# YyzHarry/imbalanced-regression

Hardware: NVIDIA B200
Metric: images/sec (higher is better)
Workload: dtype bf16

## Files before the change

### imbalanced-regression_b200/csrc/conv.cuh

```cuda
#pragma once
#include "common.cuh"

namespace dirb200 {

struct ConvShape {
  int n, h, w, cin, cout, kh, kw, stride, pad, ho, wo;
};

struct StatLayout {
  int rows, n_tiles, bn, group;
};

int conv_fprop(const __nv_bfloat16* x, const __nv_bfloat16* w, __nv_bfloat16* y, const ConvShape& s, bool stem,
               cudaStream_t st, float* stat_partial = nullptr, StatLayout* layout = nullptr);
struct ConvEpilogue {
  const float* scale;
  const float* shift;
  const __nv_bfloat16* residual;
  bool relu;
};
int conv_fprop_affine(const __nv_bfloat16* x, const __nv_bfloat16* w, __nv_bfloat16* out, const ConvShape& s,
                      const ConvEpilogue& epi, cudaStream_t st);
struct DgradBnMoments {
  const __nv_bfloat16* y;
  const float *scale, *shift;
  float* partial;
  StatLayout* layout;
};
bool conv_dgrad_fuses_bn_moments(const ConvShape& s);
int conv_dgrad(const __nv_bfloat16* dy, const __nv_bfloat16* wt, __nv_bfloat16* dx, const ConvShape& s,
               cudaStream_t st, const DgradBnMoments* bnm = nullptr);
int conv_wgrad_splits(const ConvShape& s);
size_t conv_wgrad_workspace_bytes(const ConvShape& s);
int conv_wgrad_partials(const __nv_bfloat16* x, const __nv_bfloat16* dy, float* partial, const ConvShape& s, bool stem,
                        int* splits_out, cudaStream_t st);
int wgrad_reduce(const float* workspace, int splits, float* dw, const ConvShape& s, bool stem, bool accumulate,
                 cudaStream_t st);
int conv_wgrad(const __nv_bfloat16* x, const __nv_bfloat16* dy, float* dw, float* workspace, const ConvShape& s,
               bool stem, bool accumulate, cudaStream_t st);
struct WgradReduceDesc {
  const float* partial;
  size_t w_off;
  int splits, cout, cin, kh, kw, stem;
};
int wgrad_reduce_all(const WgradReduceDesc* descs_dev, int nlayers, float* grads, cudaStream_t st);
struct PrepDesc {
  size_t w_off;
  int cout, cin, kh, kw, stem;
  __nv_bfloat16 *wf, *wd;
  FastDiv fd_cin, fd_cout, fd_taps;
// ... 17 lines not shown
```

### imbalanced-regression_b200/csrc/conv_igemm.cu

```cuda
#include <stdlib.h>
#include "common.cuh"
#include "tc.cuh"
#include "conv.cuh"

namespace dirb200 {
using namespace tc;

constexpr int BM = 128;
constexpr int BK = 64;
constexpr int kProducerThreads = 128;
constexpr int kTmaWarp = 4, kMmaWarp = 5;
constexpr int kThreads = 320;
constexpr int kMaxTaps = 25;

struct IgemmParams {
  const __nv_bfloat16* src;
  int n, hs, ws, cs;
  int hm, wm;
  int kh, kw, stride, pad;
  int transposed;
  int cls_on, cls_py, cls_px, full_h, full_w;
  int ntaps_c;
  int tap_list[kMaxTaps];
  long long tap_eoff[kMaxTaps];
  unsigned short tap_r[kMaxTaps], tap_s[kMaxTaps];
  FastDiv fd_hw, fd_wm, fd_cpb, fd_kw, fd_ntiles, fd_persplit;
  int cpb;
  long long pixels;
  int num_kblocks;
  int kblocks_per_split;
  int total_chunks;
  int m_tiles, n_tiles;
  int num_tiles;
  int a_mode;
  int i2c_stride, i2c_lo;
  int ldc;
  void* out;
  float* stat_out;
  const float* epi_scale;
  const float* epi_shift;
  const __nv_bfloat16* epi_res;
  int epi_relu;
  const __nv_bfloat16* bst_y;
  const float* bst_scale;
  const float* bst_shift;
  int patch_r, patch_wp, patch_h, patch_w;
  FastDiv fd_tpi, fd_wp;
};

template <int BN, bool STAGED_EPI, bool CTA2 = false, bool PATCH = false>
struct Cfg {
  static constexpr int kABytes = BM * BK * 2;
  static constexpr int kBRows = CTA2 ? BN / 2 : BN;
  static constexpr int kBBytes = kBRows * BK * 2;
  static constexpr int kStageBytes = PATCH ? 32768 : kABytes + kBBytes;
  static constexpr int kBresBytes = PATCH ? 9 * BN * BK * 2 : 0;
  static constexpr int kEpiCols = 64;
  static constexpr int kStages = PATCH ? 3
                                 : CTA2 ? ((BN == 256) ? 6 : 8)
                                        : (STAGED_EPI ? ((BN == 256) ? 4 : ((BN == 128) ? 6 : 8))
                                                      : ((BN == 256) ? 4 : ((BN == 128) ? 6 : 8)));
// ... 41 lines not shown
}

__device__ __forceinline__ const __nv_bfloat16* tap_source(const IgemmParams& P, const RowPre& rp, int r, int s,
                                                           int coff, bool& ok) {
  int hi, wi;
  ok = true;
  if (!P.transposed) {
    hi = rp.yb + r;
    wi = rp.xb + s;
  } else {
    hi = rp.yb - r;
    wi = rp.xb - s;
    if (P.stride == 2) {
      ok = ((hi | wi) & 1) == 0;
      hi >>= 1;
      wi >>= 1;
    }
  }
  ok = ok && static_cast<unsigned>(hi) < static_cast<unsigned>(P.hs) &&
       static_cast<unsigned>(wi) < static_cast<unsigned>(P.ws);
  return ok ? P.src + (static_cast<size_t>(rp.nb + hi) * P.ws + wi) * P.cs + coff : P.src;
}

template <int BN, bool WGRAD, bool STEM, bool CTA2 = false, bool ATMA = false, bool AFFINE = false, bool BSTAT = false,
          bool PATCH = false>
__global__ void __launch_bounds__((ATMA && !PATCH) ? kThreads - kProducerThreads : kThreads, 1)
igemm_kernel(const __grid_constant__ CUtensorMap tmap_b, const __grid_constant__ CUtensorMap tmap_a,
             const IgemmParams P) {
  using C = Cfg<BN, !WGRAD, CTA2, PATCH>;
  static_assert(!PATCH || (ATMA && !WGRAD && !CTA2 && !AFFINE && BN == 64), "patch-resident A operand: 64-wide fprop / dgrad");
  static_assert(!CTA2 || (ATMA && !WGRAD && !STEM && BN >= 128), "CTA pairs: TMA-fed fprop / dgrad GEMMs only");
  static_assert(!ATMA || !STEM, "TMA-fed A operand: not for the stem");
  static_assert(!AFFINE || (ATMA && !WGRAD), "folded-BN epilogue: TMA-fed fprop GEMMs only");
  static_assert(!BSTAT || (ATMA && !WGRAD && !AFFINE), "BN-backward moments in the epilogue: TMA-fed dgrad GEMMs only");
  extern __shared__ uint8_t smem_raw[];
  const uint32_t smem_base = (smem_u32(smem_raw) + 1023u) & ~1023u;
  const uint32_t bar_base = smem_base + C::kBarOffset;
  auto a_addr = [&](int s) { return smem_base + s * C::kStageBytes; };
  auto b_addr = [&](int s) { return smem_base + s * C::kStageBytes + C::kABytes; };
  constexpr uint32_t nstages = C::kStages;
  auto full_bar = [&](int s) { return bar_base + 8u * s; };
  auto empty_bar = [&](int s) { return bar_base + 8u * (C::kStages + s); };
  auto tfull_bar = [&](int a) { return bar_base + 8u * (2 * C::kStages + a); };
  auto tempty_bar = [&](int a) { return bar_base + 8u * (2 * C::kStages + 2 + a); };
  const uint32_t tmem_holder = bar_base + 8u * (2 * C::kStages + 4);
  const uint32_t bres_bar = bar_base + 8u * (2 * C::kStages + 5);
  const uint32_t bres_addr = smem_base + C::kBresOffset;

  const int warp = static_cast<int>(threadIdx.x >> 5) + ((ATMA && !PATCH) ? kProducerThreads / 32 : 0), lane = threadIdx.x & 31;
  const uint32_t rank = CTA2 ? cluster_ctarank() : 0u;
  const int tile_start = CTA2 ? static_cast<int>(blockIdx.x >> 1) : static_cast<int>(blockIdx.x);
// ... 603 lines not shown
      if (lane == 0) {
        if (CTA2 && rank != 0) mbar_arrive_remote(mapa_rank(tempty_bar(acc), 0));
        else mbar_arrive(tempty_bar(acc));
      }
    }
    if constexpr (!WGRAD) {
      if (P.stat_out != nullptr) {
        __syncwarp();
        if constexpr (PATCH) asm volatile("bar.sync 1, 256;" ::: "memory");
        else asm volatile("bar.sync 1, 128;" ::: "memory");
        const float* all = reinterpret_cast<const float*>(smem_raw + (smem_base - smem_u32(smem_raw)) + C::kStatOffset);
        constexpr int kWarpFloats = C::kStatWarpBytes / 4;
        float* dst = P.stat_out + static_cast<size_t>(blockIdx.x) * 2 * P.ldc + fixed_n * BN;
        if (egroup == 0) {
          for (int o = quarter * 32 + lane; o < 2 * BN; o += 128) {
            const int k = o / BN, col = o - k * BN;
            const int cb = col / C::kEpiCols, ln = (col % C::kEpiCols) >> 1, e = col & 1;
            const int idx = (cb * 4 + k * 2 + e) * 32 + ln;
            float v = (all[idx] + all[kWarpFloats + idx]) + (all[2 * kWarpFloats + idx] + all[3 * kWarpFloats + idx]);
            if constexpr (PATCH)
              v += (all[4 * kWarpFloats + idx] + all[5 * kWarpFloats + idx]) + (all[6 * kWarpFloats + idx] + all[7 * kWarpFloats + idx]);
            dst[static_cast<size_t>(k) * P.ldc + col] = v;
          }
        }
      }
    }
  }

  tcgen05_fence_before();
  __syncwarp();
  if constexpr (CTA2) cluster_sync_all();
  else __syncthreads();
  if (warp == kMmaWarp) {
    tcgen05_fence_after();
    if constexpr (CTA2) tmem_dealloc_cta2(tmem_base, C::kTmemCols);
    else tmem_dealloc(tmem_base, C::kTmemCols);
  }
}


constexpr int kWgpThreads = 192;
constexpr int kWgpStages = 4, kWgpASlot = 32768, kWgpBSlot = 16384, kWgpStage = kWgpASlot + kWgpBSlot;
constexpr int kWgpSmemBytes = kWgpStages * kWgpStage + 256 + 1024;

__global__ void __launch_bounds__(kWgpThreads, 1)
wgrad_patch_kernel(const __grid_constant__ CUtensorMap tmap_x, const __grid_constant__ CUtensorMap tmap_dy,
                   const IgemmParams P) {
  extern __shared__ uint8_t smem_raw[];
  const uint32_t smem_base = (smem_u32(smem_raw) + 1023u) & ~1023u;
  const uint32_t bar_base = smem_base + kWgpStages * kWgpStage;
  auto a_addr = [&](int s) { return smem_base + s * kWgpStage; };
  auto b_addr = [&](int s) { return smem_base + s * kWgpStage + kWgpASlot; };
  auto full_bar = [&](int s) { return bar_base + 8u * s; };
  auto empty_bar = [&](int s) { return bar_base + 8u * (kWgpStages + s); };
  const uint32_t done_bar = bar_base + 8u * (2 * kWgpStages), tmem_holder = bar_base + 8u * (2 * kWgpStages + 1);
  const int warp = threadIdx.x >> 5, lane = threadIdx.x & 31;

  for (int i = threadIdx.x; i < kWgpStages * kWgpStage / 16; i += kWgpThreads)
    asm volatile("st.shared.v4.b32 [%0], {%1, %1, %1, %1};" ::"r"(smem_base + i * 16), "r"(0u) : "memory");
// ... 389 lines not shown
    set_error("cuTensorMapEncodeTiled (patch) failed (%d) w=%d h=%d n=%d rows=%d", (int)cr, w, h, n, box_rows);
    return DIRB200_ERR_CUDA;
  }
  return DIRB200_OK;
}

static int launch_patch(const __nv_bfloat16* src, const __nv_bfloat16* wmat, IgemmParams P, int n, int h, int w, int r,
                        bool flipped, cudaStream_t st) {
  CUtensorMap ta, tb;
  if (int rc = make_tmap_patch(&ta, src, n, h, w, r + 2)) return rc;
  if (int rc = make_tmap_bf16_2d(&tb, wmat, 9 * 64, 64, 9 * 64 * 2, 64)) return rc;
  P.patch_r = r; P.patch_wp = w + 2; P.patch_h = h; P.patch_w = w;
  P.transposed = flipped ? 1 : 0;
  P.a_mode = 3;
  P.n_tiles = 1;
  P.m_tiles = n * (h / r);
  P.num_tiles = P.m_tiles;
  P.num_kblocks = 9;
  if (P.bst_y != nullptr) return launch_igemm_impl<64, false, false, true, false, true, true>(tb, ta, P, st);
  return launch_igemm_impl<64, false, false, true, false, false, true>(tb, ta, P, st);
}

static int conv_fprop_impl(const __nv_bfloat16* x, const __nv_bfloat16* w, __nv_bfloat16* y, const ConvShape& s, bool stem,
                           cudaStream_t st, float* stat_partial, const ConvEpilogue* epi);

int conv_fprop(const __nv_bfloat16* x, const __nv_bfloat16* w, __nv_bfloat16* y, const ConvShape& s, bool stem,
               cudaStream_t st, float* stat_partial, StatLayout* layout) {
  const int rc = conv_fprop_impl(x, w, y, s, stem, st, stat_partial, nullptr);
  if (layout) *layout = t_last_layout;
  return rc;
}

int conv_fprop_affine(const __nv_bfloat16* x, const __nv_bfloat16* w, __nv_bfloat16* out, const ConvShape& s,
                      const ConvEpilogue& epi, cudaStream_t st) {
  DIRB_CHECK_ARG(epi.scale && epi.shift, "conv_fprop_affine: scale / shift missing");
  return conv_fprop_impl(x, w, out, s, false, st, nullptr, &epi);
}

static int conv_fprop_impl(const __nv_bfloat16* x, const __nv_bfloat16* w, __nv_bfloat16* y, const ConvShape& s, bool stem,
                           cudaStream_t st, float* stat_partial, const ConvEpilogue* epi) {
  if (int rc = check_shape(s, stem, "conv_fprop")) return rc;
  const int ktot = s.kh * s.kw * s.cin;
  IgemmParams P{};
  P.src = x; P.n = s.n; P.hs = s.h; P.ws = s.w; P.cs = s.cin; P.hm = s.ho; P.wm = s.wo;
  P.kh = s.kh; P.kw = s.kw; P.stride = s.stride; P.pad = s.pad; P.transposed = 0;
  P.cpb = stem ? 1 : s.cin / 64;
  P.pixels = static_cast<long long>(s.n) * s.ho * s.wo;
  P.num_kblocks = ktot / 64;
  P.ntaps_c = s.kh * s.kw;
  DIRB_CHECK_ARG(stem || P.ntaps_c <= kMaxTaps, "conv_fprop: at most %d filter taps (got %dx%d)", kMaxTaps, s.kh, s.kw);
  for (int i = 0; i < kMaxTaps; ++i) P.tap_list[i] = i;
  P.ldc = s.cout; P.out = y;
  P.stat_out = stat_partial;
  if (epi) {
    P.epi_scale = epi->scale; P.epi_shift = epi->shift; P.epi_res = epi->residual; P.epi_relu = epi->relu ? 1 : 0;
  }
  if (!stem && !epi) {
    if (const int pr = patch_rows(s.h, s.w, s.cin, s.kh, s.kw, s.stride, s.pad, s.cout))
      return launch_patch(x, w, P, s.n, s.h, s.w, pr, false, st);
  }
  const int m_tiles = static_cast<int>((P.pixels + BM - 1) / BM);
  const int bn = pick_bn(s.cout, m_tiles, !is_plain_gemm(s, stem));
  P.n_tiles = s.cout / bn;
  CUtensorMap tm, ta;
  bool tma_fed = false;
  if (is_plain_gemm(s, stem)) {
    if (int rc = make_tmap_bf16_2d(&ta, x, s.cin, static_cast<uint64_t>(P.pixels), static_cast<uint64_t>(s.cin) * 2, BM))
      return rc;
    P.a_mode = 1;
    tma_fed = true;
  } else if (!stem && im2col_enabled()) {
    if (int rc = make_tmap_im2col_bf16(&ta, x, s.cin, s.w, s.h, s.n, -s.pad, -s.pad, s.pad - (s.kw - 1),
                                       s.pad - (s.kh - 1), s.stride, BM))
      return rc;
    P.a_mode = 2; P.i2c_stride = s.stride; P.i2c_lo = -s.pad;
    tma_fed = true;
  }
  if (tma_fed && want_pairs(bn, P.num_kblocks)) return launch_cta2(w, ktot, s.cout, P, m_tiles, st, ta);
  if (int rc = make_tmap_bf16_2d(&tm, w, ktot, s.cout, static_cast<uint64_t>(ktot) * 2, bn)) return rc;
  if (stem) return DISPATCH_BN(bn, false, true, tm, P, m_tiles, 1, st);
  if (tma_fed) return DISPATCH_BN(bn, false, false, tm, P, m_tiles, 1, st, &ta);
  return DISPATCH_BN(bn, false, false, tm, P, m_tiles, 1, st);
}

bool conv_dgrad_fuses_bn_moments(const ConvShape& s) {
  return s.stride == 1 && (is_plain_gemm(s, false) || (im2col_enabled() && s.kh == s.kw));
}

int conv_dgrad(const __nv_bfloat16* dy, const __nv_bfloat16* wt, __nv_bfloat16* dx, const ConvShape& s,
               cudaStream_t st, const DgradBnMoments* bnm) {
  if (int rc = check_shape(s, false, "conv_dgrad")) return rc;
  DIRB_CHECK_ARG(!bnm || (conv_dgrad_fuses_bn_moments(s) && bnm->y && bnm->scale && bnm->shift && bnm->partial),
                 "conv_dgrad: BN-backward moments are fused into TMA-fed stride-1 dgrads only");
  DIRB_CHECK_ARG(s.stride == 1 || s.stride == 2, "conv_dgrad: stride must be 1 or 2 (got %d)", s.stride);
  DIRB_CHECK_ARG(s.kh * s.kw <= (s.stride == 1 ? kMaxTaps : 9), "conv_dgrad: at most %d filter taps (stride 2: 9; got %dx%d)",
                 kMaxTaps, s.kh, s.kw);
  const int ktot = s.kh * s.kw * s.cout;
  IgemmParams P{};
  P.src = dy; P.n = s.n; P.hs = s.ho; P.ws = s.wo; P.cs = s.cout; P.hm = s.h; P.wm = s.w;
  P.kh = s.kh; P.kw = s.kw; P.stride = s.stride; P.pad = s.pad; P.transposed = 1;
  P.cpb = s.cout / 64;
  P.ldc = s.cin; P.out = dx;
  if (bnm) {
    P.bst_y = bnm->y; P.bst_scale = bnm->scale; P.bst_shift = bnm->shift; P.stat_out = bnm->partial;
  }
  CUtensorMap tm;
  if (s.stride == 1) {
    P.pixels = static_cast<long long>(s.n) * s.h * s.w;
    P.ntaps_c = s.kh * s.kw;
    for (int i = 0; i < kMaxTaps; ++i) P.tap_list[i] = i;
    P.num_kblocks = ktot / 64;
    if (const int pr = patch_rows(s.ho, s.wo, s.cout, s.kh, s.kw, s.stride, s.pad, s.cin)) {
      const int rc = launch_patch(dy, wt, P, s.n, s.ho, s.wo, pr, true, st);
      if (bnm && bnm->layout) *bnm->layout = t_last_layout;
      return rc;
    }
    const int m_tiles = static_cast<int>((P.pixels + BM - 1) / BM);
    const int bn = pick_bn(s.cin, m_tiles, !is_plain_gemm(s, false));
    P.n_tiles = s.cin / bn;
    CUtensorMap ta;
    bool tma_fed = false;
    if (is_plain_gemm(s, false)) {
      if (int rc = make_tmap_bf16_2d(&ta, dy, s.cout, static_cast<uint64_t>(P.pixels), static_cast<uint64_t>(s.cout) * 2, BM))
        return rc;
      P.a_mode = 1;
      tma_fed = true;
    } else if (im2col_enabled() && s.kh == s.kw) {
// ... 217 lines not shown
```

### imbalanced-regression_b200/csrc/nn_kernels.cu

```cuda
#include "common.cuh"
#include "conv.cuh"
#include "nn.cuh"

namespace dirb200 {

constexpr int kReduceCtasPerSm = 4;

struct V8 {
  float v[8];
};
__device__ __forceinline__ V8 load8(const __nv_bfloat16* p) {
  const uint4 u = *reinterpret_cast<const uint4*>(p);
  const __nv_bfloat162* h = reinterpret_cast<const __nv_bfloat162*>(&u);
  V8 r;
#pragma unroll
  for (int i = 0; i < 4; ++i) {
    const float2 f = __bfloat1622float2(h[i]);
    r.v[2 * i] = f.x;
    r.v[2 * i + 1] = f.y;
  }
  return r;
}
__device__ __forceinline__ void store8(__nv_bfloat16* p, const V8& a) {
  uint4 u;
  __nv_bfloat162* h = reinterpret_cast<__nv_bfloat162*>(&u);
// ... 77 lines not shown
#pragma unroll
    for (int u = 0; u < 4; ++u) x[u] = load8(y + (r + u * stride) * c + cg * 8);
#pragma unroll
    for (int u = 0; u < 4; ++u)
#pragma unroll
      for (int j = 0; j < 8; ++j) {
        acc[0][j] += x[u].v[j];
        acc[1][j] = fmaf(x[u].v[j], x[u].v[j], acc[1][j]);
      }
  }
  for (; r < rows; r += stride) {
    const V8 x = load8(y + r * c + cg * 8);
#pragma unroll
    for (int j = 0; j < 8; ++j) {
      acc[0][j] += x.v[j];
      acc[1][j] = fmaf(x.v[j], x.v[j], acc[1][j]);
    }
  }
  column_reduce_finish<2>(acc, cg, cgroups, c, partial);
}

__device__ __forceinline__ void sum_layout2(const float* __restrict__ partial, const StatLayout& L, int c, int i,
                                            double (*sh)[32][32], double& r0, double& r1) {
  double a0 = 0.0, b0 = 0.0, a1 = 0.0, b1 = 0.0;
  if (i < c) {
    const int j = i / L.bn;
    const int ngroups = L.rows / L.group;
    const int nk = j < ngroups ? (ngroups - 1 - j) / L.n_tiles + 1 : 0;
    const int nrows = nk * L.group;
    int t = threadIdx.y;
    for (; t + 32 < nrows; t += 64) {
      const int q0 = (j + (t / L.group) * L.n_tiles) * L.group + t % L.group;
      const int q1 = (j + ((t + 32) / L.group) * L.n_tiles) * L.group + (t + 32) % L.group;
      const float x0 = partial[((size_t)q0 * 2) * c + i], y0 = partial[((size_t)q0 * 2 + 1) * c + i];
      const float x1 = partial[((size_t)q1 * 2) * c + i], y1 = partial[((size_t)q1 * 2 + 1) * c + i];
      a0 += (double)x0; b0 += (double)y0; a1 += (double)x1; b1 += (double)y1;
    }
    if (t < nrows) {
      const int q0 = (j + (t / L.group) * L.n_tiles) * L.group + t % L.group;
      a0 += (double)partial[((size_t)q0 * 2) * c + i];
      b0 += (double)partial[((size_t)q0 * 2 + 1) * c + i];
    }
  }
  sh[0][threadIdx.y][threadIdx.x] = a0 + a1;
  sh[1][threadIdx.y][threadIdx.x] = b0 + b1;
  __syncthreads();
  r0 = r1 = 0.0;
  if (threadIdx.y == 0)
    for (int w = 0; w < 32; ++w) {
      r0 += sh[0][w][threadIdx.x];
      r1 += sh[1][w][threadIdx.x];
    }
}

__global__ void bn_finalize_kernel(const float* __restrict__ partial, StatLayout L, int64_t rows, int c,
                                   const float* __restrict__ gamma, const float* __restrict__ beta, float eps,
                                   float momentum, float* __restrict__ running_mean, float* __restrict__ running_var,
                                   float* __restrict__ mean_out, float* __restrict__ invstd_out,
                                   float* __restrict__ scale, float* __restrict__ shift) {
  __shared__ double sh[2][32][32];
  const int i = blockIdx.x * 32 + threadIdx.x;
  double sx, sq;
  sum_layout2(partial, L, c, i, sh, sx, sq);
  if (threadIdx.y != 0 || i >= c) return;
  const double n = (double)rows;
  const double m = sx / n;
  double var = sq / n - m * m;
  if (var < 0.0) var = 0.0;
  const float invstd = (float)(1.0 / sqrt(var + (double)eps));
  mean_out[i] = (float)m;
  invstd_out[i] = invstd;
  const float sc = gamma[i] * invstd;
  scale[i] = sc;
  shift[i] = beta[i] - (float)m * sc;
  if (running_mean) {
    const double unbiased = rows > 1 ? var * n / (n - 1.0) : var;
    running_mean[i] = (1.f - momentum) * running_mean[i] + momentum * (float)m;
    running_var[i] = (1.f - momentum) * running_var[i] + momentum * (float)unbiased;
  }
}

__global__ void bn_eval_coeffs_kernel(int c, const float* __restrict__ gamma, const float* __restrict__ beta, float eps,
                                      const float* __restrict__ running_mean, const float* __restrict__ running_var,
                                      float* __restrict__ scale, float* __restrict__ shift) {
  const int i = blockIdx.x * blockDim.x + threadIdx.x;
  if (i >= c) return;
  const float sc = gamma[i] * rsqrtf(running_var[i] + eps);
  scale[i] = sc;
  shift[i] = beta[i] - running_mean[i] * sc;
}

__global__ void bn_eval_coeffs_all_kernel(const BnEvalDesc* __restrict__ descs, const float* __restrict__ params,
                                          const float* __restrict__ running, float eps) {
  const BnEvalDesc d = descs[blockIdx.y];
  const int i = blockIdx.x * blockDim.x + threadIdx.x;
  if (i >= d.c) return;
  const float sc = params[d.gamma_off + i] * rsqrtf(running[d.rv_off + i] + eps);
  d.scale[i] = sc;
  d.shift[i] = params[d.beta_off + i] - running[d.rm_off + i] * sc;
}

__device__ __forceinline__ uint32_t f2_to_bf2(float a, float b) {
// ... 166 lines not shown
        const float2 yv = bf2_to_f2(yw[w]);
        ms.apply(M[u], w, yv, g);
        if (WRITE_DZ) {
          oz[w] = f2_to_bf2(g.x, g.y);
          g = bf2_to_f2(oz[w]);
        }
        acc[0][2 * w] += g.x;
        acc[0][2 * w + 1] += g.y;
        acc[1][2 * w] = fmaf(g.x, yv.x, acc[1][2 * w]);
        acc[1][2 * w + 1] = fmaf(g.y, yv.y, acc[1][2 * w + 1]);
        if (HAS_Y2) {
          const uint32_t y2w[4] = {Y2[u].x, Y2[u].y, Y2[u].z, Y2[u].w};
          const float2 y2v = bf2_to_f2(y2w[w]);
          acc[K - 1][2 * w] = fmaf(g.x, y2v.x, acc[K - 1][2 * w]);
          acc[K - 1][2 * w + 1] = fmaf(g.y, y2v.y, acc[K - 1][2 * w + 1]);
        }
      }
      if (WRITE_DZ) *reinterpret_cast<uint4*>(dz_out + (u ? o1 : o0)) = make_uint4(oz[0], oz[1], oz[2], oz[3]);
    }
  }
  column_reduce_finish<K>(acc, cg, cgroups, c, partial);
}

__device__ __forceinline__ void bn_bwd_coeffs_write(double db, double s1, int i, int64_t rows, int c,
                                                    const float* __restrict__ mean, const float* __restrict__ invstd,
                                                    const float* __restrict__ gamma, float* __restrict__ grad_gamma,
                                                    float* __restrict__ grad_beta, float* __restrict__ coef) {
  const double n = (double)rows, is = (double)invstd[i], ga = (double)gamma[i], mu = (double)mean[i];
  const double dg = is * (s1 - mu * db);
  coef[i] = (float)(ga * is);
  coef[c + i] = (float)(-ga * is * is * dg / n);
  coef[2 * c + i] = (float)(ga * is * (mu * is * dg / n - db / n));
  grad_gamma[i] += (float)dg;
  grad_beta[i] += (float)db;
}

__global__ void bn_bwd_coeffs_kernel(const float* __restrict__ partial, int nblocks, int K, int gslot, int64_t rows,
                                     int c, const float* __restrict__ mean, const float* __restrict__ invstd,
                                     const float* __restrict__ gamma, float* __restrict__ grad_gamma,
                                     float* __restrict__ grad_beta, float* __restrict__ coef ) {
  __shared__ double sh[32][32];
  const int i = blockIdx.x * 32 + threadIdx.x;
  double db, s1;
  sum_partials2(partial, nblocks, K, 0, gslot, c, i, sh, db, s1);
  if (threadIdx.y != 0 || i >= c) return;
  bn_bwd_coeffs_write(db, s1, i, rows, c, mean, invstd, gamma, grad_gamma, grad_beta, coef);
}

__global__ void bn_bwd_coeffs_layout_kernel(const float* __restrict__ partial, StatLayout L, int64_t rows, int c,
                                            const float* __restrict__ mean, const float* __restrict__ invstd,
                                            const float* __restrict__ gamma, float* __restrict__ grad_gamma,
                                            float* __restrict__ grad_beta, float* __restrict__ coef) {
  __shared__ double sh[2][32][32];
  const int i = blockIdx.x * 32 + threadIdx.x;
  double db, s1;
  sum_layout2(partial, L, c, i, sh, db, s1);
  if (threadIdx.y != 0 || i >= c) return;
  bn_bwd_coeffs_write(db, s1, i, rows, c, mean, invstd, gamma, grad_gamma, grad_beta, coef);
}
// ... 781 lines not shown
```

### imbalanced-regression_b200/csrc/resnet_runner.cu

```cuda
#include <stdlib.h>
#include <vector>
#include "common.cuh"
#include "conv.cuh"
#include "nn.cuh"

namespace dirb200 {

struct BNLayer {
  int c = 0;
  size_t gamma_off = 0, beta_off = 0;
  size_t rm_off = 0, rv_off = 0;
  float *mean = nullptr, *invstd = nullptr, *scale = nullptr, *shift = nullptr, *coef = nullptr;
};

struct ConvLayer {
  ConvShape s{};
  bool stem = false;
  size_t w_off = 0;
  __nv_bfloat16 *wf = nullptr, *wd = nullptr;
  float* wpart = nullptr;
  __nv_bfloat16* y = nullptr;
  __nv_bfloat16* a = nullptr;
  int64_t rows = 0;
  BNLayer bn;
// ... 4 lines not shown
  bool has_ds = false;
  const __nv_bfloat16* in = nullptr;
  __nv_bfloat16* out = nullptr;
  uint8_t* mask = nullptr;
};

}

using namespace dirb200;

struct dirb200_net {
  int n = 0, h = 0, w = 0;
  ConvLayer stem;
  std::vector<Block> blocks;
  __nv_bfloat16 *x_s2d = nullptr, *pool_out = nullptr;
  uint8_t* pool_idx = nullptr;
  int pool_h = 0, pool_w = 0;
  int feat_c = 0, feat_hw = 0;
  __nv_bfloat16* scratch[8] = {};
  WgradReduceDesc* reduce_descs = nullptr;
  std::vector<int> reduce_begin;
  float* bn_partial = nullptr;
  float* stat_partial = nullptr;
  PrepDesc* prep_descs = nullptr;
  BnEvalDesc* bn_eval_descs = nullptr;
  int num_bns = 0, max_bn_c = 0;
  int num_convs = 0;
  size_t param_count = 0, running_count = 0, activation_bytes = 0;
  std::vector<void*> allocs;
  bool forward_was_training = false;
  std::vector<int> stage_begin;
  int bwd_next_stage = -1;
  __nv_bfloat16 *bw_gA = nullptr, *bw_gB = nullptr, *bw_nA = nullptr, *bw_nB = nullptr, *bw_spareB = nullptr;
  int bw_gB_h = 0, bw_gB_w = 0;
  struct GraphSlot {
    cudaGraphExec_t exec = nullptr;
    const void *k0 = nullptr, *k1 = nullptr;
    int warm = 0;
    int64_t launches = 0;
    __nv_bfloat16 *gA = nullptr, *gB = nullptr, *nA = nullptr, *nB = nullptr, *spareB = nullptr;
    int gB_h = 0, gB_w = 0;
  };
  GraphSlot g_fwd, g_bwd[6];
  cudaStream_t cap_stream = nullptr;
  float *enc_buf = nullptr, *denc_buf = nullptr;
  bool profiling = false;
// ... 99 lines not shown
      rd.push_back(WgradReduceDesc{cv.wpart, cv.w_off, conv_wgrad_splits(cv.s), cv.s.cout, cv.stem ? 3 : cv.s.cin,
                                   cv.stem ? 7 : cv.s.kh, cv.stem ? 7 : cv.s.kw, cv.stem ? 1 : 0});
    };
    net->reduce_begin.clear();
    net->reduce_begin.push_back(0);
    addr(net->stem);
    for (int stg = 1; stg <= num_stages; ++stg) {
      net->reduce_begin.push_back((int)rd.size());
      for (int bi = net->stage_begin[stg]; bi < net->stage_begin[stg + 1]; ++bi) {
        Block& B = net->blocks[bi];
        addr(B.c1); addr(B.c2); addr(B.c3);
        if (B.has_ds) addr(B.ds);
      }
    }
    net->reduce_begin.push_back((int)rd.size());
    NET_ALLOC(net->reduce_descs, sizeof(WgradReduceDesc) * rd.size());
    if (cudaMemcpy(net->reduce_descs, rd.data(), sizeof(WgradReduceDesc) * rd.size(), cudaMemcpyHostToDevice) != cudaSuccess)
      return false;
  }
  NET_ALLOC(net->enc_buf, sizeof(float) * (size_t)n * net->feat_c);
  NET_ALLOC(net->denc_buf, sizeof(float) * (size_t)n * net->feat_c);
  NET_ALLOC(net->bn_partial, sizeof(float) * bn_partial_floats(net->feat_c));
  NET_ALLOC(net->stat_partial, sizeof(float) * bn_partial_floats(net->feat_c));
  std::vector<PrepDesc> descs;
  auto add = [&](const ConvLayer& cv) {
    descs.push_back(make_prep_desc(cv.w_off, cv.s.cout, cv.stem ? 3 : cv.s.cin, cv.stem ? 7 : cv.s.kh, cv.stem ? 7 : cv.s.kw,
                                   cv.stem ? 1 : 0, cv.wf, cv.wd));
  };
  add(net->stem);
  for (Block& B : net->blocks) {
    add(B.c1); add(B.c2); add(B.c3);
    if (B.has_ds) add(B.ds);
  }
  net->num_convs = (int)descs.size();
  NET_ALLOC(net->prep_descs, sizeof(PrepDesc) * descs.size());
  if (cudaMemcpy(net->prep_descs, descs.data(), sizeof(PrepDesc) * descs.size(), cudaMemcpyHostToDevice) != cudaSuccess)
    return false;
  std::vector<BnEvalDesc> bd;
  auto addbn = [&](const BNLayer& bn) {
    bd.push_back(BnEvalDesc{bn.c, bn.gamma_off, bn.beta_off, bn.rm_off, bn.rv_off, bn.scale, bn.shift});
    net->max_bn_c = std::max(net->max_bn_c, bn.c);
  };
  addbn(net->stem.bn);
  for (Block& B : net->blocks) {
    addbn(B.c1.bn); addbn(B.c2.bn); addbn(B.c3.bn);
    if (B.has_ds) addbn(B.ds.bn);
// ... 27 lines not shown
  cudaEventRecord(r.a, st);
  net->prof.push_back(r);
}
static inline void prof_end(dirb200_net* net, cudaStream_t st) {
  if (!net->profiling) return;
  cudaEventRecord(net->prof.back().b, st);
}
#define RUNP(kind, expr)          \
  do {                            \
    prof_begin(net, (kind), st);  \
    int _rc = (expr);             \
    prof_end(net, st);            \
    if (_rc) return _rc;          \
  } while (0)

static bool fused_stats() {
  static const bool on = [] {
    const char* e = getenv("DIRB200_FUSED_STATS");
    return !(e != nullptr && e[0] == '0');
  }();
  return on;
}

static int conv_bn_forward(dirb200_net* net, ConvLayer& cv, const __nv_bfloat16* in, const float* params,
                           float* running, bool training, cudaStream_t st) {
  BNLayer& bn = cv.bn;
  if (training) {
    StatLayout lay{};
    const bool fused = fused_stats();
    RUNP(kFprop, conv_fprop(in, cv.wf, cv.y, cv.s, cv.stem, st, fused ? net->stat_partial : nullptr, &lay));
    if (!fused) {
      int nblk = 0;
      RUNP(kBnStats, bn_stats(cv.y, cv.rows, bn.c, net->stat_partial, &nblk, st));
      lay = StatLayout{nblk, 1, bn.c, 1};
    }
    RUNP(kBnStats, bn_finalize(net->stat_partial, lay, cv.rows, bn.c, params + bn.gamma_off, params + bn.beta_off, 1e-5f,
                               0.1f, running ? running + bn.rm_off : nullptr, running ? running + bn.rv_off : nullptr,
                               bn.mean, bn.invstd, bn.scale, bn.shift, st));
  } else {
    RUNP(kFprop, conv_fprop(in, cv.wf, cv.y, cv.s, cv.stem, st));
    RUNP(kBnStats, bn_eval_coeffs(bn.c, params + bn.gamma_off, params + bn.beta_off, 1e-5f, running + bn.rm_off,
                                  running + bn.rv_off, bn.scale, bn.shift, st));
  }
  if (cv.a)
    RUNP(kBnApply, bn_apply(cv.y, bn.scale, bn.shift, nullptr, nullptr, nullptr, nullptr, true, cv.rows, bn.c, cv.a, nullptr, st));
  return DIRB200_OK;
}

static int wgrad_step(dirb200_net* net, const __nv_bfloat16* x, const __nv_bfloat16* dy, ConvLayer& cv, cudaStream_t st) {
  int splits = 1;
  RUNP(kWgrad, conv_wgrad_partials(x, dy, cv.wpart, cv.s, cv.stem, &splits, st));
  return DIRB200_OK;
}

static int wgrad_reduce_stage(dirb200_net* net, int stage, float* grads, cudaStream_t st) {
  const int lo = net->reduce_begin[stage], hi = net->reduce_begin[stage + 1];
  RUNP(kWgradReduce, wgrad_reduce_all(net->reduce_descs + lo, hi - lo, grads, st));
  return DIRB200_OK;
}

static int conv_bn_backward(dirb200_net* net, ConvLayer& cv, const __nv_bfloat16* g, const float* params, float* grads,
                            __nv_bfloat16* dy, cudaStream_t st, const StatLayout* moments = nullptr) {
  BNLayer& bn = cv.bn;
  if (moments) {
    RUNP(kBnBwdApply, bn_bwd_coeffs_layout(net->bn_partial, *moments, cv.rows, bn.c, bn.mean, bn.invstd,
                                           params + bn.gamma_off, grads + bn.gamma_off, grads + bn.beta_off, bn.coef, st));
  } else {
    int nblk = 0;
    RUNP(kBnBwdReduce, bn_bwd_reduce(g, nullptr, cv.y, nullptr, bn.scale, bn.shift, nullptr, cv.rows, bn.c,
                                     net->bn_partial, &nblk, st));
    RUNP(kBnBwdApply, bn_bwd_coeffs(net->bn_partial, nblk, 2, 1, cv.rows, bn.c, bn.mean, bn.invstd,
                                    params + bn.gamma_off, grads + bn.gamma_off, grads + bn.beta_off, bn.coef, st));
  }
  RUNP(kBnBwdApply, bn_bwd_apply(g, nullptr, cv.y, bn.coef, nullptr, nullptr, bn.scale, bn.shift, nullptr, cv.rows, bn.c,
                                 dy, nullptr, nullptr, st));
  return DIRB200_OK;
}

static bool folded_eval() {
  static const bool on = [] {
    const char* e = getenv("DIRB200_FOLDED_EVAL");
    return !(e != nullptr && e[0] == '0');
  }();
  return on;
}

static int forward_eval_folded(dirb200_net* net, const float* params, const float* running, float* enc_out,
                               cudaStream_t st) {
  RUNP(kBnStats, bn_eval_coeffs_all(net->bn_eval_descs, net->num_bns, net->max_bn_c, params, running, 1e-5f, st));
  RUNP(kFprop, conv_fprop(net->x_s2d, net->stem.wf, net->stem.y, net->stem.s, true, st));
// ... 54 lines not shown
  g.launches = g_launches.load() - before;
  g_launches.fetch_sub(g.launches);
  const cudaError_t ei = cudaGraphInstantiate(&g.exec, graph, 0);
  cudaGraphDestroy(graph);
  if (ei != cudaSuccess) {
    g.exec = nullptr;
    set_error("resnet: cudaGraphInstantiate failed (%s)", cudaGetErrorString(ei));
    return DIRB200_ERR_CUDA;
  }
  DIRB_CUDA(cudaGraphLaunch(g.exec, st));
  g_launches.fetch_add(g.launches);
  return DIRB200_OK;
}

static bool fused_bwd_moments() {
  static const bool on = [] {
    const char* e = getenv("DIRB200_FUSED_BWD_MOMENTS");
    return !(e != nullptr && e[0] == '0');
  }();
  return on;
}

static int dgrad_with_bn_moments(dirb200_net* net, const __nv_bfloat16* dy, ConvLayer& cv, ConvLayer& prev,
                                 __nv_bfloat16* g, StatLayout* lay, bool* fused, cudaStream_t st) {
  *fused = fused_bwd_moments() && conv_dgrad_fuses_bn_moments(cv.s);
  if (!*fused) {
    RUNP(kDgrad, conv_dgrad(dy, cv.wd, g, cv.s, st));
    return DIRB200_OK;
  }
  const DgradBnMoments bm{prev.y, prev.bn.scale, prev.bn.shift, net->bn_partial, lay};
  RUNP(kDgrad, conv_dgrad(dy, cv.wd, g, cv.s, st, &bm));
  return DIRB200_OK;
}

}

extern "C" {

int dirb200_resnet_create(int n, int h, int w, const int* blocks_per_stage, int num_stages, dirb200_net** out) {
  DIRB_CHECK_ARG(out && blocks_per_stage && n > 0 && num_stages >= 1 && num_stages <= 4, "resnet_create: bad arguments");
  DIRB_CHECK_ARG(h > 0 && w > 0 && h % 32 == 0 && w % 32 == 0, "resnet_create: H and W must be multiples of 32");
  dirb200_net* net = new dirb200_net();
  net->n = n; net->h = h; net->w = w;
  if (!build(net, blocks_per_stage, num_stages)) {
    for (void* p : net->allocs) cudaFree(p);
    delete net;
    return DIRB200_ERR_CUDA;
  }
  *out = net;
  return DIRB200_OK;
}

void dirb200_resnet_destroy(dirb200_net* net) {
// ... 91 lines not shown
    Block& B = net->blocks[bi];
    BNLayer& b3 = B.c3.bn;
    int nblk = 0;
    const int kparts = B.has_ds ? 3 : 2;
    RUNP(kBnBwdReduce, bn_bwd_reduce(gA, gB, B.c3.y, B.has_ds ? B.ds.y : nullptr, nullptr, nullptr, B.mask, B.c3.rows,
                                     b3.c, net->bn_partial, &nblk, st, gB_h, gB_w, B.has_ds ? nullptr : nB));
    if (B.has_ds) {
      BNLayer& bd = B.ds.bn;
      RUNP(kBnBwdApply, bn_bwd_coeffs(net->bn_partial, nblk, kparts, 2, B.c3.rows, b3.c, bd.mean, bd.invstd,
                                      params + bd.gamma_off, grads + bd.gamma_off, grads + bd.beta_off, bd.coef, st));
    }
    RUNP(kBnBwdApply, bn_bwd_coeffs(net->bn_partial, nblk, kparts, 1, B.c3.rows, b3.c, b3.mean, b3.invstd,
                                    params + b3.gamma_off, grads + b3.gamma_off, grads + b3.beta_off, b3.coef, st));
    if (B.has_ds)
      RUNP(kBnBwdApply, bn_bwd_apply(gA, gB, B.c3.y, b3.coef, B.ds.y, B.ds.bn.coef, nullptr, nullptr, B.mask, B.c3.rows,
                                     b3.c, t1, t2, nullptr, st, gB_h, gB_w));
    else
      RUNP(kBnBwdApply, bn_bwd_apply(nB, nullptr, B.c3.y, b3.coef, nullptr, nullptr, nullptr, nullptr, nullptr, B.c3.rows,
                                     b3.c, t1, nullptr, nullptr, st));
    gB_h = gB_w = 0;
    RUN(wgrad_step(net, B.c2.a, t1, B.c3, st));
    StatLayout mlay{};
    bool mfused = false;
    RUN(dgrad_with_bn_moments(net, t1, B.c3, B.c2, t3, &mlay, &mfused, st));
    RUN(conv_bn_backward(net, B.c2, t3, params, grads, t1, st, mfused ? &mlay : nullptr));
    RUN(wgrad_step(net, B.c1.a, t1, B.c2, st));
    RUN(dgrad_with_bn_moments(net, t1, B.c2, B.c1, t3, &mlay, &mfused, st));
    RUN(conv_bn_backward(net, B.c1, t3, params, grads, t1, st, mfused ? &mlay : nullptr));
    RUN(wgrad_step(net, B.in, t1, B.c1, st));
    RUNP(kDgrad, conv_dgrad(t1, B.c1.wd, nA, B.c1.s, st));
    if (B.has_ds) {
      RUN(wgrad_step(net, B.in, t2, B.ds, st));
      const ConvShape& d = B.ds.s;
      if (d.stride == 2 && d.kh == 1 && d.kw == 1 && d.pad == 0 && d.h % 2 == 0 && d.w % 2 == 0 && bi > 0 &&
          !net->blocks[bi - 1].has_ds) {
        const ConvShape cs{d.n, d.ho, d.wo, d.cin, d.cout, 1, 1, 1, 0, d.ho, d.wo};
        RUNP(kDgrad, conv_dgrad(t2, B.ds.wd, nB, cs, st));
        gB_h = d.h;
        gB_w = d.w;
      } else {
        RUNP(kDgrad, conv_dgrad(t2, B.ds.wd, nB, B.ds.s, st));
      }
    }
    __nv_bfloat16* oldA = gA;
    __nv_bfloat16* oldB = gB ? gB : spareB;
    gA = nA; gB = nB;
    nA = oldA; nB = oldB;
    spareB = nullptr;
  }
  net->bw_gA = gA; net->bw_gB = gB; net->bw_nA = nA; net->bw_nB = nB; net->bw_spareB = spareB;
  net->bw_gB_h = gB_h; net->bw_gB_w = gB_w;
// ... 111 lines not shown
```

Baseline: 14340.

## Fold BN statistics finalize into conv epilogue via last-CTA ticket

Adds a last-arriving-CTA tail to the implicit-GEMM conv kernel. Each CTA bumps an atomic ticket per column tile, and the final CTA reduces the per-tile BN partial sums and writes the mean, invstd, scale and shift (forward) or the backward coefficients and gamma/beta grads (dgrad). This removes the separate bn_finalize and bn_bwd_coeffs launches and one read pass over the partials. In exchange it adds a threadfence, an atomic, and a serial tail reduction in one CTA per column tile, which can lengthen the kernel's critical path.

```diff
diff --git a/imbalanced-regression_b200/csrc/bn_coeffs.cuh b/imbalanced-regression_b200/csrc/bn_coeffs.cuh
--- /dev/null
+++ b/imbalanced-regression_b200/csrc/bn_coeffs.cuh
@@ -0,0 +1,77 @@
+#pragma once
+#include "common.cuh"
+#include "conv.cuh"
+
+namespace dirb200 {
+
+__device__ __forceinline__ int stat_row(const StatLayout& L, int j, int k) {
+  return (j + (k / L.group) * L.n_tiles) * L.group + k % L.group;
+}
+__device__ __forceinline__ int stat_tile_rows(const StatLayout& L, int j) {
+  const int ngroups = L.rows / L.group;
+  return (j < ngroups ? (ngroups - 1 - j) / L.n_tiles + 1 : 0) * L.group;
+}
+
+template <typename Load>
+__device__ __forceinline__ void stat_lane_sums(int nrows, int t, const Load& load, double& r0, double& r1) {
+  double a0 = 0.0, b0 = 0.0, a1 = 0.0, b1 = 0.0;
+  int k = t;
+  for (; k + 32 < nrows; k += 64) {
+    float x0, y0, x1, y1;
+    load(k, x0, y0);
+    load(k + 32, x1, y1);
+    a0 += (double)x0; b0 += (double)y0; a1 += (double)x1; b1 += (double)y1;
+  }
+  if (k < nrows) {
+    float x0, y0;
+    load(k, x0, y0);
+    a0 += (double)x0;
+    b0 += (double)y0;
+  }
+  r0 = a0 + a1;
+  r1 = b0 + b1;
+}
+
+__device__ __forceinline__ double stat_combine(const double* lane, int stride) {
+  double r = 0.0;
+  for (int w = 0; w < 32; ++w) r += lane[w * stride];
+  return r;
+}
+
+__device__ __forceinline__ void bn_finalize_write(double sx, double sq, int i, int64_t rows,
+                                                  const float* __restrict__ gamma, const float* __restrict__ beta,
+                                                  float eps, float momentum, float* __restrict__ running_mean,
+                                                  float* __restrict__ running_var, float* __restrict__ mean_out,
+                                                  float* __restrict__ invstd_out, float* __restrict__ scale,
+                                                  float* __restrict__ shift) {
+  const double n = (double)rows;
+  const double m = sx / n;
+  double var = sq / n - m * m;
+  if (var < 0.0) var = 0.0;
+  const float invstd = (float)(1.0 / sqrt(var + (double)eps));
+  mean_out[i] = (float)m;
+  invstd_out[i] = invstd;
+  const float sc = gamma[i] * invstd;
+  scale[i] = sc;
+  shift[i] = beta[i] - (float)m * sc;
+  if (running_mean) {
+    const double unbiased = rows > 1 ? var * n / (n - 1.0) : var;
+    running_mean[i] = (1.f - momentum) * running_mean[i] + momentum * (float)m;
+    running_var[i] = (1.f - momentum) * running_var[i] + momentum * (float)unbiased;
+  }
+}
+
+__device__ __forceinline__ void bn_bwd_coeffs_write(double db, double s1, int i, int64_t rows, int c,
+                                                    const float* __restrict__ mean, const float* __restrict__ invstd,
+                                                    const float* __restrict__ gamma, float* __restrict__ grad_gamma,
+                                                    float* __restrict__ grad_beta, float* __restrict__ coef) {
+  const double n = (double)rows, is = (double)invstd[i], ga = (double)gamma[i], mu = (double)mean[i];
+  const double dg = is * (s1 - mu * db);
+  coef[i] = (float)(ga * is);
+  coef[c + i] = (float)(-ga * is * is * dg / n);
+  coef[2 * c + i] = (float)(ga * is * (mu * is * dg / n - db / n));
+  grad_gamma[i] += (float)dg;
+  grad_beta[i] += (float)db;
+}
+
+}
diff --git a/imbalanced-regression_b200/csrc/conv.cuh b/imbalanced-regression_b200/csrc/conv.cuh
--- a/imbalanced-regression_b200/csrc/conv.cuh
+++ b/imbalanced-regression_b200/csrc/conv.cuh
@@ -11,8 +11,22 @@
   int rows, n_tiles, bn, group;
 };
 
+struct BnFoldFwd {
+  unsigned* ticket;
+  const float *gamma, *beta;
+  float eps, momentum;
+  float *running_mean, *running_var;
+  float *mean, *invstd, *scale, *shift;
+};
+struct BnFoldBwd {
+  unsigned* ticket;
+  const float *mean, *invstd, *gamma;
+  float *grad_gamma, *grad_beta, *coef;
+};
+
 int conv_fprop(const __nv_bfloat16* x, const __nv_bfloat16* w, __nv_bfloat16* y, const ConvShape& s, bool stem,
-               cudaStream_t st, float* stat_partial = nullptr, StatLayout* layout = nullptr);
+               cudaStream_t st, float* stat_partial = nullptr, StatLayout* layout = nullptr,
+               const BnFoldFwd* fold = nullptr);
 struct ConvEpilogue {
   const float* scale;
   const float* shift;
@@ -26,6 +40,7 @@
   const float *scale, *shift;
   float* partial;
   StatLayout* layout;
+  const BnFoldBwd* fold;
 };
 bool conv_dgrad_fuses_bn_moments(const ConvShape& s);
 int conv_dgrad(const __nv_bfloat16* dy, const __nv_bfloat16* wt, __nv_bfloat16* dx, const ConvShape& s,
diff --git a/imbalanced-regression_b200/csrc/conv_igemm.cu b/imbalanced-regression_b200/csrc/conv_igemm.cu
--- a/imbalanced-regression_b200/csrc/conv_igemm.cu
+++ b/imbalanced-regression_b200/csrc/conv_igemm.cu
@@ -2,6 +2,7 @@
 #include "common.cuh"
 #include "tc.cuh"
 #include "conv.cuh"
+#include "bn_coeffs.cuh"
 
 namespace dirb200 {
 using namespace tc;
@@ -37,6 +38,8 @@
   int ldc;
   void* out;
   float* stat_out;
+  BnFoldFwd fold_fwd;
+  BnFoldBwd fold_bwd;
   const float* epi_scale;
   const float* epi_shift;
   const __nv_bfloat16* epi_res;
@@ -124,11 +127,63 @@
   return ok ? P.src + (static_cast<size_t>(rp.nb + hi) * P.ws + wi) * P.cs + coff : P.src;
 }
 
+template <int BN, bool BSTAT, int GROUP>
+__device__ __noinline__ void bn_fold_tail(const IgemmParams& P, int j, int* last_flag, float* stage,
+                                             uint32_t stage_bytes) {
+  unsigned* ticket = BSTAT ? P.fold_bwd.ticket : P.fold_fwd.ticket;
+  const StatLayout L{static_cast<int>(gridDim.x), P.n_tiles, BN, GROUP};
+  const int nrows = stat_tile_rows(L, j);
+  if (threadIdx.x == 0) *last_flag = atomicAdd(ticket + j, 1u) + 1u == static_cast<unsigned>(nrows);
+  __syncthreads();
+  if (!*last_flag) return;
+  __threadfence();
+  const int c = P.ldc, c0 = j * BN;
+  int cw = BN;
+  while (cw > 4 && static_cast<uint32_t>(nrows) * 8u * cw > stage_bytes) cw >>= 1;
+  const int pieces = cw / 4;
+  const uint32_t stage_s = smem_u32(stage);
+  for (int cs = 0; cs < BN; cs += cw) {
+    for (int p = threadIdx.x; p < nrows * 2 * pieces; p += blockDim.x) {
+      const int k = p / (2 * pieces), rem = p - k * 2 * pieces;
+      const size_t q = static_cast<size_t>(stat_row(L, j, k));
+      const int slot = rem / pieces, piece = rem - slot * pieces;
+      cp_async16(stage_s + static_cast<uint32_t>(((k * 2 + slot) * cw + piece * 4) * 4),
+                 P.stat_out + (q * 2 + slot) * c + c0 + cs + piece * 4, 16u);
+    }
+    cp_async_commit();
+    cp_async_wait<0>();
+    __syncthreads();
+    for (int cc = threadIdx.x; cc < cw; cc += blockDim.x) {
+      double r0 = 0.0, r1 = 0.0;
+      for (int t = 0; t < 32; ++t) {
+        double v0, v1;
+        stat_lane_sums(nrows, t, [&](int k, float& x0, float& x1) {
+          x0 = stage[(k * 2) * cw + cc];
+          x1 = stage[(k * 2 + 1) * cw + cc];
+        }, v0, v1);
+        r0 += v0;
+        r1 += v1;
+      }
+      const int ch = c0 + cs + cc;
+      if constexpr (BSTAT) {
+        const BnFoldBwd& F = P.fold_bwd;
+        bn_bwd_coeffs_write(r0, r1, ch, P.pixels, c, F.mean, F.invstd, F.gamma, F.grad_gamma, F.grad_beta, F.coef);
+      } else {
+        const BnFoldFwd& F = P.fold_fwd;
+        bn_finalize_write(r0, r1, ch, P.pixels, F.gamma, F.beta, F.eps, F.momentum, F.running_mean, F.running_var,
+                          F.mean, F.invstd, F.scale, F.shift);
+      }
+    }
+    __syncthreads();
+  }
+  if (threadIdx.x == 0) ticket[j] = 0u;
+}
+
 template <int BN, bool WGRAD, bool STEM, bool CTA2 = false, bool ATMA = false, bool AFFINE = false, bool BSTAT = false,
           bool PATCH = false>
 __global__ void __launch_bounds__((ATMA && !PATCH) ? kThreads - kProducerThreads : kThreads, 1)
 igemm_kernel(const __grid_constant__ CUtensorMap tmap_b, const __grid_constant__ CUtensorMap tmap_a,
-             const IgemmParams P) {
+             const __grid_constant__ IgemmParams P) {
   using C = Cfg<BN, !WGRAD, CTA2, PATCH>;
   static_assert(!PATCH || (ATMA && !WGRAD && !CTA2 && !AFFINE && BN == 64), "patch-resident A operand: 64-wide fprop / dgrad");
   static_assert(!CTA2 || (ATMA && !WGRAD && !STEM && BN >= 128), "CTA pairs: TMA-fed fprop / dgrad GEMMs only");
@@ -778,6 +833,7 @@
               v += (all[4 * kWarpFloats + idx] + all[5 * kWarpFloats + idx]) + (all[6 * kWarpFloats + idx] + all[7 * kWarpFloats + idx]);
             dst[static_cast<size_t>(k) * P.ldc + col] = v;
           }
+          if ((BSTAT ? P.fold_bwd.ticket : P.fold_fwd.ticket) != nullptr) __threadfence();
         }
       }
     }
@@ -791,6 +847,15 @@
     tcgen05_fence_after();
     if constexpr (CTA2) tmem_dealloc_cta2(tmem_base, C::kTmemCols);
     else tmem_dealloc(tmem_base, C::kTmemCols);
+  }
+  if constexpr (!WGRAD) {
+    if (P.stat_out != nullptr && (BSTAT ? P.fold_bwd.ticket : P.fold_fwd.ticket) != nullptr) {
+      bn_fold_tail<BN, BSTAT, CTA2 ? 2 : 1>(P, fixed_n,
+                                             reinterpret_cast<int*>(smem_raw + (bar_base - smem_u32(smem_raw)) +
+                                                                    8u * (2 * C::kStages + 6)),
+                                             reinterpret_cast<float*>(smem_raw + (smem_base - smem_u32(smem_raw))),
+                                             static_cast<uint32_t>(C::kBresOffset));
+    }
   }
 }
 
@@ -1226,11 +1291,14 @@
 }
 
 static int conv_fprop_impl(const __nv_bfloat16* x, const __nv_bfloat16* w, __nv_bfloat16* y, const ConvShape& s, bool stem,
-                           cudaStream_t st, float* stat_partial, const ConvEpilogue* epi);
+                           cudaStream_t st, float* stat_partial, const ConvEpilogue* epi, const BnFoldFwd* fold);
 
 int conv_fprop(const __nv_bfloat16* x, const __nv_bfloat16* w, __nv_bfloat16* y, const ConvShape& s, bool stem,
-               cudaStream_t st, float* stat_partial, StatLayout* layout) {
-  const int rc = conv_fprop_impl(x, w, y, s, stem, st, stat_partial, nullptr);
+               cudaStream_t st, float* stat_partial, StatLayout* layout, const BnFoldFwd* fold) {
+  DIRB_CHECK_ARG(!fold || (stat_partial && fold->ticket && fold->gamma && fold->beta && fold->mean && fold->invstd &&
+                           fold->scale && fold->shift && !fold->running_mean == !fold->running_var),
+                 "conv_fprop: a statistics finalize needs the statistics buffer, a ticket and every output");
+  const int rc = conv_fprop_impl(x, w, y, s, stem, st, stat_partial, nullptr, fold);
   if (layout) *layout = t_last_layout;
   return rc;
 }
@@ -1238,11 +1306,11 @@
 int conv_fprop_affine(const __nv_bfloat16* x, const __nv_bfloat16* w, __nv_bfloat16* out, const ConvShape& s,
                       const ConvEpilogue& epi, cudaStream_t st) {
   DIRB_CHECK_ARG(epi.scale && epi.shift, "conv_fprop_affine: scale / shift missing");
-  return conv_fprop_impl(x, w, out, s, false, st, nullptr, &epi);
+  return conv_fprop_impl(x, w, out, s, false, st, nullptr, &epi, nullptr);
 }
 
 static int conv_fprop_impl(const __nv_bfloat16* x, const __nv_bfloat16* w, __nv_bfloat16* y, const ConvShape& s, bool stem,
-                           cudaStream_t st, float* stat_partial, const ConvEpilogue* epi) {
+                           cudaStream_t st, float* stat_partial, const ConvEpilogue* epi, const BnFoldFwd* fold) {
   if (int rc = check_shape(s, stem, "conv_fprop")) return rc;
   const int ktot = s.kh * s.kw * s.cin;
   IgemmParams P{};
@@ -1256,6 +1324,7 @@
   for (int i = 0; i < kMaxTaps; ++i) P.tap_list[i] = i;
   P.ldc = s.cout; P.out = y;
   P.stat_out = stat_partial;
+  if (fold) P.fold_fwd = *fold;
   if (epi) {
     P.epi_scale = epi->scale; P.epi_shift = epi->shift; P.epi_res = epi->residual; P.epi_relu = epi->relu ? 1 : 0;
   }
@@ -1296,6 +1365,9 @@
   if (int rc = check_shape(s, false, "conv_dgrad")) return rc;
   DIRB_CHECK_ARG(!bnm || (conv_dgrad_fuses_bn_moments(s) && bnm->y && bnm->scale && bnm->shift && bnm->partial),
                  "conv_dgrad: BN-backward moments are fused into TMA-fed stride-1 dgrads only");
+  DIRB_CHECK_ARG(!bnm || !bnm->fold || (bnm->fold->ticket && bnm->fold->mean && bnm->fold->invstd && bnm->fold->gamma &&
+                                        bnm->fold->grad_gamma && bnm->fold->grad_beta && bnm->fold->coef),
+                 "conv_dgrad: a BN-backward coefficient fold needs a ticket and every input / output");
   DIRB_CHECK_ARG(s.stride == 1 || s.stride == 2, "conv_dgrad: stride must be 1 or 2 (got %d)", s.stride);
   DIRB_CHECK_ARG(s.kh * s.kw <= (s.stride == 1 ? kMaxTaps : 9), "conv_dgrad: at most %d filter taps (stride 2: 9; got %dx%d)",
                  kMaxTaps, s.kh, s.kw);
@@ -1307,6 +1379,7 @@
   P.ldc = s.cin; P.out = dx;
   if (bnm) {
     P.bst_y = bnm->y; P.bst_scale = bnm->scale; P.bst_shift = bnm->shift; P.stat_out = bnm->partial;
+    if (bnm->fold) P.fold_bwd = *bnm->fold;
   }
   CUtensorMap tm;
   if (s.stride == 1) {
diff --git a/imbalanced-regression_b200/csrc/nn_kernels.cu b/imbalanced-regression_b200/csrc/nn_kernels.cu
--- a/imbalanced-regression_b200/csrc/nn_kernels.cu
+++ b/imbalanced-regression_b200/csrc/nn_kernels.cu
@@ -1,6 +1,7 @@
 #include "common.cuh"
 #include "conv.cuh"
 #include "nn.cuh"
+#include "bn_coeffs.cuh"
 
 namespace dirb200 {
 
@@ -124,35 +125,23 @@
 
 __device__ __forceinline__ void sum_layout2(const float* __restrict__ partial, const StatLayout& L, int c, int i,
                                             double (*sh)[32][32], double& r0, double& r1) {
-  double a0 = 0.0, b0 = 0.0, a1 = 0.0, b1 = 0.0;
+  double a = 0.0, b = 0.0;
   if (i < c) {
     const int j = i / L.bn;
-    const int ngroups = L.rows / L.group;
-    const int nk = j < ngroups ? (ngroups - 1 - j) / L.n_tiles + 1 : 0;
-    const int nrows = nk * L.group;
-    int t = threadIdx.y;
-    for (; t + 32 < nrows; t += 64) {
-      const int q0 = (j + (t / L.group) * L.n_tiles) * L.group + t % L.group;
-      const int q1 = (j + ((t + 32) / L.group) * L.n_tiles) * L.group + (t + 32) % L.group;
-      const float x0 = partial[((size_t)q0 * 2) * c + i], y0 = partial[((size_t)q0 * 2 + 1) * c + i];
-      const float x1 = partial[((size_t)q1 * 2) * c + i], y1 = partial[((size_t)q1 * 2 + 1) * c + i];
-      a0 += (double)x0; b0 += (double)y0; a1 += (double)x1; b1 += (double)y1;
-    }
-    if (t < nrows) {
-      const int q0 = (j + (t / L.group) * L.n_tiles) * L.group + t % L.group;
-      a0 += (double)partial[((size_t)q0 * 2) * c + i];
-      b0 += (double)partial[((size_t)q0 * 2 + 1) * c + i];
-    }
-  }
-  sh[0][threadIdx.y][threadIdx.x] = a0 + a1;
-  sh[1][threadIdx.y][threadIdx.x] = b0 + b1;
+    stat_lane_sums(stat_tile_rows(L, j), threadIdx.y, [&](int k, float& x0, float& x1) {
+      const size_t q = static_cast<size_t>(stat_row(L, j, k));
+      x0 = partial[(q * 2) * c + i];
+      x1 = partial[(q * 2 + 1) * c + i];
+    }, a, b);
+  }
+  sh[0][threadIdx.y][threadIdx.x] = a;
+  sh[1][threadIdx.y][threadIdx.x] = b;
   __syncthreads();
   r0 = r1 = 0.0;
-  if (threadIdx.y == 0)
-    for (int w = 0; w < 32; ++w) {
-      r0 += sh[0][w][threadIdx.x];
-      r1 += sh[1][w][threadIdx.x];
-    }
+  if (threadIdx.y == 0) {
+    r0 = stat_combine(&sh[0][0][threadIdx.x], 32);
+    r1 = stat_combine(&sh[1][0][threadIdx.x], 32);
+  }
 }
 
 __global__ void bn_finalize_kernel(const float* __restrict__ partial, StatLayout L, int64_t rows, int c,
@@ -165,21 +154,8 @@
   double sx, sq;
   sum_layout2(partial, L, c, i, sh, sx, sq);
   if (threadIdx.y != 0 || i >= c) return;
-  const double n = (double)rows;
-  const double m = sx / n;
-  double var = sq / n - m * m;
-  if (var < 0.0) var = 0.0;
-  const float invstd = (float)(1.0 / sqrt(var + (double)eps));
-  mean_out[i] = (float)m;
-  invstd_out[i] = invstd;
-  const float sc = gamma[i] * invstd;
-  scale[i] = sc;
-  shift[i] = beta[i] - (float)m * sc;
-  if (running_mean) {
-    const double unbiased = rows > 1 ? var * n / (n - 1.0) : var;
-    running_mean[i] = (1.f - momentum) * running_mean[i] + momentum * (float)m;
-    running_var[i] = (1.f - momentum) * running_var[i] + momentum * (float)unbiased;
-  }
+  bn_finalize_write(sx, sq, i, rows, gamma, beta, eps, momentum, running_mean, running_var, mean_out, invstd_out, scale,
+                    shift);
 }
 
 __global__ void bn_eval_coeffs_kernel(int c, const float* __restrict__ gamma, const float* __restrict__ beta, float eps,
@@ -392,19 +368,6 @@
   column_reduce_finish<K>(acc, cg, cgroups, c, partial);
 }
 
-__device__ __forceinline__ void bn_bwd_coeffs_write(double db, double s1, int i, int64_t rows, int c,
-                                                    const float* __restrict__ mean, const float* __restrict__ invstd,
-                                                    const float* __restrict__ gamma, float* __restrict__ grad_gamma,
-                                                    float* __restrict__ grad_beta, float* __restrict__ coef) {
-  const double n = (double)rows, is = (double)invstd[i], ga = (double)gamma[i], mu = (double)mean[i];
-  const double dg = is * (s1 - mu * db);
-  coef[i] = (float)(ga * is);
-  coef[c + i] = (float)(-ga * is * is * dg / n);
-  coef[2 * c + i] = (float)(ga * is * (mu * is * dg / n - db / n));
-  grad_gamma[i] += (float)dg;
-  grad_beta[i] += (float)db;
-}
-
 __global__ void bn_bwd_coeffs_kernel(const float* __restrict__ partial, int nblocks, int K, int gslot, int64_t rows,
                                      int c, const float* __restrict__ mean, const float* __restrict__ invstd,
                                      const float* __restrict__ gamma, float* __restrict__ grad_gamma,
diff --git a/imbalanced-regression_b200/csrc/resnet_runner.cu b/imbalanced-regression_b200/csrc/resnet_runner.cu
--- a/imbalanced-regression_b200/csrc/resnet_runner.cu
+++ b/imbalanced-regression_b200/csrc/resnet_runner.cu
@@ -50,6 +50,7 @@
   std::vector<int> reduce_begin;
   float* bn_partial = nullptr;
   float* stat_partial = nullptr;
+  unsigned* fold_tickets = nullptr;
   PrepDesc* prep_descs = nullptr;
   BnEvalDesc* bn_eval_descs = nullptr;
   int num_bns = 0, max_bn_c = 0;
@@ -195,6 +196,8 @@
   NET_ALLOC(net->denc_buf, sizeof(float) * (size_t)n * net->feat_c);
   NET_ALLOC(net->bn_partial, sizeof(float) * bn_partial_floats(net->feat_c));
   NET_ALLOC(net->stat_partial, sizeof(float) * bn_partial_floats(net->feat_c));
+  NET_ALLOC(net->fold_tickets, sizeof(unsigned) * 2 * (net->feat_c / 64));
+  if (cudaMemset(net->fold_tickets, 0, sizeof(unsigned) * 2 * (net->feat_c / 64)) != cudaSuccess) return false;
   std::vector<PrepDesc> descs;
   auto add = [&](const ConvLayer& cv) {
     descs.push_back(make_prep_desc(cv.w_off, cv.s.cout, cv.stem ? 3 : cv.s.cin, cv.stem ? 7 : cv.s.kh, cv.stem ? 7 : cv.s.kw,
@@ -268,12 +271,30 @@
   return on;
 }
 
+static bool fold_bn_coeffs() {
+  static const bool on = [] {
+    const char* e = getenv("DIRB200_FOLD_BN_COEFFS");
+    return !(e != nullptr && e[0] == '0');
+  }();
+  return on;
+}
+
 static int conv_bn_forward(dirb200_net* net, ConvLayer& cv, const __nv_bfloat16* in, const float* params,
                            float* running, bool training, cudaStream_t st) {
   BNLayer& bn = cv.bn;
   if (training) {
     StatLayout lay{};
     const bool fused = fused_stats();
+    if (fused && fold_bn_coeffs()) {
+      const BnFoldFwd fold{net->fold_tickets, params + bn.gamma_off, params + bn.beta_off, 1e-5f, 0.1f,
+                           running ? running + bn.rm_off : nullptr, running ? running + bn.rv_off : nullptr,
+                           bn.mean, bn.invstd, bn.scale, bn.shift};
+      RUNP(kFprop, conv_fprop(in, cv.wf, cv.y, cv.s, cv.stem, st, net->stat_partial, &lay, &fold));
+      if (cv.a)
+        RUNP(kBnApply, bn_apply(cv.y, bn.scale, bn.shift, nullptr, nullptr, nullptr, nullptr, true, cv.rows, bn.c, cv.a,
+                                nullptr, st));
+      return DIRB200_OK;
+    }
     RUNP(kFprop, conv_fprop(in, cv.wf, cv.y, cv.s, cv.stem, st, fused ? net->stat_partial : nullptr, &lay));
     if (!fused) {
       int nblk = 0;
@@ -306,12 +327,13 @@
 }
 
 static int conv_bn_backward(dirb200_net* net, ConvLayer& cv, const __nv_bfloat16* g, const float* params, float* grads,
-                            __nv_bfloat16* dy, cudaStream_t st, const StatLayout* moments = nullptr) {
+                            __nv_bfloat16* dy, cudaStream_t st, const StatLayout* moments = nullptr,
+                            bool coef_ready = false) {
   BNLayer& bn = cv.bn;
-  if (moments) {
+  if (moments && !coef_ready) {
     RUNP(kBnBwdApply, bn_bwd_coeffs_layout(net->bn_partial, *moments, cv.rows, bn.c, bn.mean, bn.invstd,
                                            params + bn.gamma_off, grads + bn.gamma_off, grads + bn.beta_off, bn.coef, st));
-  } else {
+  } else if (!moments) {
     int nblk = 0;
     RUNP(kBnBwdReduce, bn_bwd_reduce(g, nullptr, cv.y, nullptr, bn.scale, bn.shift, nullptr, cv.rows, bn.c,
                                      net->bn_partial, &nblk, st));
@@ -412,13 +434,17 @@
 }
 
 static int dgrad_with_bn_moments(dirb200_net* net, const __nv_bfloat16* dy, ConvLayer& cv, ConvLayer& prev,
-                                 __nv_bfloat16* g, StatLayout* lay, bool* fused, cudaStream_t st) {
+                                 const float* params, float* grads, __nv_bfloat16* g, StatLayout* lay, bool* fused,
+                                 cudaStream_t st) {
   *fused = fused_bwd_moments() && conv_dgrad_fuses_bn_moments(cv.s);
   if (!*fused) {
     RUNP(kDgrad, conv_dgrad(dy, cv.wd, g, cv.s, st));
     return DIRB200_OK;
   }
-  const DgradBnMoments bm{prev.y, prev.bn.scale, prev.bn.shift, net->bn_partial, lay};
+  const BNLayer& pb = prev.bn;
+  const BnFoldBwd fold{net->fold_tickets + net->feat_c / 64, pb.mean, pb.invstd, params + pb.gamma_off,
+                       grads + pb.gamma_off, grads + pb.beta_off, pb.coef};
+  const DgradBnMoments bm{prev.y, pb.scale, pb.shift, net->bn_partial, lay, fold_bn_coeffs() ? &fold : nullptr};
   RUNP(kDgrad, conv_dgrad(dy, cv.wd, g, cv.s, st, &bm));
   return DIRB200_OK;
 }
@@ -556,11 +582,11 @@
     RUN(wgrad_step(net, B.c2.a, t1, B.c3, st));
     StatLayout mlay{};
     bool mfused = false;
-    RUN(dgrad_with_bn_moments(net, t1, B.c3, B.c2, t3, &mlay, &mfused, st));
-    RUN(conv_bn_backward(net, B.c2, t3, params, grads, t1, st, mfused ? &mlay : nullptr));
+    RUN(dgrad_with_bn_moments(net, t1, B.c3, B.c2, params, grads, t3, &mlay, &mfused, st));
+    RUN(conv_bn_backward(net, B.c2, t3, params, grads, t1, st, mfused ? &mlay : nullptr, mfused && fold_bn_coeffs()));
     RUN(wgrad_step(net, B.c1.a, t1, B.c2, st));
-    RUN(dgrad_with_bn_moments(net, t1, B.c2, B.c1, t3, &mlay, &mfused, st));
-    RUN(conv_bn_backward(net, B.c1, t3, params, grads, t1, st, mfused ? &mlay : nullptr));
+    RUN(dgrad_with_bn_moments(net, t1, B.c2, B.c1, params, grads, t3, &mlay, &mfused, st));
+    RUN(conv_bn_backward(net, B.c1, t3, params, grads, t1, st, mfused ? &mlay : nullptr, mfused && fold_bn_coeffs()));
     RUN(wgrad_step(net, B.in, t1, B.c1, st));
     RUNP(kDgrad, conv_dgrad(t1, B.c1.wd, nA, B.c1.s, st));
     if (B.has_ds) {
```

After: 13440, median of 6. 6.2% lower.
